# francescoalemanno/KissABC.jl

Hardware: AMD Instinct MI355X
Metric: walker proposal+cost evals/sec at N=65536 walkers, D=8 (higher is better)
Workload: dtype f64

## Files before the change

### include/kabc.h

```cpp
#ifndef KABC_H
#define KABC_H

#ifndef __HIPCC_RTC__
#include <stddef.h>
#include <stdint.h>
#else
#include "kabc_rtc_types.h"
#endif

#ifdef __cplusplus
extern "C" {
#endif

#define KABC_VERSION 321
#define KABC_MAX_DIM 16
#define KABC_MAX_DIM_DYN 256

typedef enum kabc_status {
    KABC_OK = 0,
    KABC_ERR_INVALID_ARG = 1,
    KABC_ERR_RETRY_EXHAUSTED = 2,
    KABC_ERR_INVALID_STATE = 3,
    KABC_ERR_DEVICE = 4,
    KABC_ERR_UNSUPPORTED = 5,
// ... 101 lines not shown

typedef struct kabc_reject_result {
    double* theta;
    double* cost;
    double* logprior;
    int64_t* index;
    int64_t capacity;
    int64_t n_out;
    int64_t draws;
    int64_t accepted_seen;
    double eps;
    int32_t exhausted;
    int32_t course;
    int64_t launches;
    double kernel_ms;
} kabc_reject_result_t;

void kabc_reject_default_opts(kabc_reject_opts_t* opts);
kabc_status_t kabc_abc_reject(kabc_ctx_t* ctx, const kabc_prior_t* prior, int32_t D, const kabc_cost_t* cost,
                              const kabc_reject_opts_t* opts, kabc_reject_result_t* result);

kabc_status_t kabc_abc_reject_batch(kabc_ctx_t* ctx, const kabc_prior_t* prior, int32_t D,
                                    const kabc_cost_t* costs, int64_t nruns, const uint64_t* seeds,
                                    const double* eps, const kabc_reject_opts_t* opts,
                                    kabc_reject_result_t* results, kabc_status_t* status);
void kabc_reject_batch_stats(int64_t out[4]);

kabc_status_t kabc_math_probe(kabc_ctx_t* ctx, int32_t fn, int64_t n, const double* x,
                              double* out);

kabc_status_t kabc_ais_wide_deal(const int32_t* simd, int32_t waves, int32_t chunk, int32_t nc,
                                 uint32_t* masks);
void kabc_ais_wide_shipped(int32_t geom[3]);

enum {
    KABC_PREBUILT_AIS_HALF = 1,
    KABC_PREBUILT_AIS_WIDE = 2,
    KABC_PREBUILT_AIS_SMALL = 3,
    KABC_PREBUILT_SMC_PHASES = 4,
    KABC_PREBUILT_SMC_LOOP = 5,
    KABC_PREBUILT_SMC_SMALL = 6,
    KABC_PREBUILT_ABCDE_GEN = 7,
    KABC_PREBUILT_ABCDE_SMALL = 8,
    KABC_PREBUILT_PF_PHASES = 9,
    KABC_PREBUILT_PF_SMALL = 10,
    KABC_PREBUILT_PF_BATCH = 11
};
int32_t kabc_prebuilt_has(int32_t family, int32_t cost_id, int32_t D, int32_t variant);
void kabc_ctx_last_kernel(kabc_ctx_t* ctx, int32_t info[6]);

kabc_status_t kabc_poison_probe(kabc_ctx_t* ctx, int64_t n, uint8_t* fresh, uint8_t* pooled,
                                uint8_t* recycled, int32_t info[2]);

kabc_status_t kabc_register_cost_plugin(const char* path, int32_t* out_cost_id);
kabc_status_t kabc_compile_cost_plugin(const char* src, const int32_t* dims, int32_t ndims,
                                       int32_t posterior_mask, int32_t* out_cost_id);
kabc_status_t kabc_plugin_precompile(int32_t cost_id, int32_t family, int32_t D, int32_t variant);

kabc_status_t kabc_compile_prior_plugin(const char* src, int32_t discrete, int32_t* out_kind);

kabc_status_t kabc_compile_mvprior_plugin(const char* src, int32_t* out_kind);

#define KABC_FAMILY_AIS 1
#define KABC_FAMILY_SMC 2
#define KABC_FAMILY_ABCDE 4
#define KABC_FAMILY_PFILTER 8
// ... 322 lines not shown
```

### kissabc.jl_amd/_cdefs.py

```python
import ctypes as C

KABC_MAX_DIM = 16
KABC_MAX_DIM_DYN = 256
KABC_VERSION = 321
KABC_COMM_ID_BYTES = 128
KABC_MAX_EXCHANGE_CHUNKS = 16
KABC_COMM_MAX_WORLD = 16
COMM_RCCL, COMM_P2P = 1, 2

KABC_OK, KABC_ERR_INVALID_ARG, KABC_ERR_RETRY_EXHAUSTED, KABC_ERR_INVALID_STATE, \
    KABC_ERR_DEVICE, KABC_ERR_UNSUPPORTED, KABC_ERR_NAN_COST, KABC_ERR_CANCELLED = range(8)

PRIOR_UNIFORM, PRIOR_NORMAL, PRIOR_TRUNCNORMAL, PRIOR_BETA, PRIOR_DISCRETE_UNIFORM, \
    PRIOR_NEGBINOMIAL, PRIOR_EXPONENTIAL, PRIOR_GAMMA, PRIOR_LOGNORMAL = range(1, 10)
PRIOR_USER_INIT = 10
PRIOR_MVNORMAL = 11
PRIOR_USER = 100
FAMILY_AIS, FAMILY_SMC, FAMILY_ABCDE, FAMILY_PFILTER, FAMILY_AIS_SMALL = 1, 2, 4, 8, 16

POSTERIOR_KERNELIZED, POSTERIOR_THRESHOLD, POSTERIOR_COMMON = 1, 2, 3
SUMMARY_AUTO, SUMMARY_FULL, SUMMARY_DIAG = 0, 1, 2
KABC_AUTOCORR_MAX_LAG = 256
KABC_HIST_MAX_BINS = 1024

# ... 97 lines not shown
                ("seed", C.c_uint64), ("first_row", C.c_int64)]


class RejectResult(C.Structure):
    _fields_ = [("theta", c_double_p), ("cost", c_double_p), ("logprior", c_double_p),
                ("index", C.POINTER(C.c_int64)), ("capacity", C.c_int64), ("n_out", C.c_int64),
                ("draws", C.c_int64), ("accepted_seen", C.c_int64), ("eps", C.c_double),
                ("exhausted", C.c_int32), ("course", C.c_int32), ("launches", C.c_int64),
                ("kernel_ms", C.c_double)]


ABI_REJECT_OPTS, ABI_REJECT_RESULT = 32, 33

VP = C.c_void_p
PROTOTYPES = {
    "kabc_version": (C.c_int32, []),
    "kabc_abi_sizeof": (C.c_int32, [C.c_int32]),
    "kabc_abi_offsetof": (C.c_int32, [C.c_int32, C.c_int32]),
    "kabc_mvnormal_register": (C.c_int, [c_double_p, c_double_p, C.c_int32, C.POINTER(C.c_int32)]),
    "kabc_last_error": (C.c_char_p, []),
    "kabc_device_count": (C.c_int32, []),
    "kabc_ctx_create": (C.c_int, [C.c_int32, VP, C.POINTER(VP)]),
    "kabc_ctx_destroy": (C.c_int, [VP]),
    "kabc_ctx_synchronize": (C.c_int, [VP]),
    "kabc_ctx_cancel": (C.c_int, [VP]),
    "kabc_ctx_clear_cancel": (C.c_int, [VP]),
    "kabc_ctx_cancel_on_sigint": (C.c_int, [VP, C.c_int32]),
    "kabc_math_probe": (C.c_int, [VP, C.c_int32, C.c_int64, c_double_p, c_double_p]),
    "kabc_poison_probe": (C.c_int, [VP, C.c_int64, C.POINTER(C.c_uint8), C.POINTER(C.c_uint8),
                                    C.POINTER(C.c_uint8), C.POINTER(C.c_int32)]),
    "kabc_ais_wide_deal": (C.c_int, [C.POINTER(C.c_int32), C.c_int32, C.c_int32, C.c_int32,
                                     C.POINTER(C.c_uint32)]),
    "kabc_ais_wide_shipped": (None, [C.POINTER(C.c_int32)]),
    "kabc_prebuilt_has": (C.c_int32, [C.c_int32, C.c_int32, C.c_int32, C.c_int32]),
    "kabc_ctx_last_kernel": (None, [VP, C.POINTER(C.c_int32)]),
    "kabc_host_alloc": (C.c_int, [C.c_size_t, C.POINTER(VP)]),
    "kabc_host_free": (C.c_int, [VP]),
    "kabc_factored_logpdf": (C.c_int, [VP, C.POINTER(Prior), C.c_int32, C.c_int64, c_double_p,
                                       c_double_p]),
    "kabc_factored_push_p": (C.c_int, [VP, C.POINTER(Prior), C.c_int32, C.c_int64, c_double_p,
                                       c_double_p]),
    "kabc_factored_rand": (C.c_int, [VP, C.POINTER(Prior), C.c_int32, C.c_uint64, C.c_uint32,
                                     C.c_int64, C.c_int64, C.c_uint64, c_double_p]),
    "kabc_cost_eval": (C.c_int, [VP, C.POINTER(Cost), C.c_int32, C.c_int64, c_double_p, C.c_int32,
                                 C.c_uint64, C.c_int64, c_double_p]),
    "kabc_prior_predictive": (C.c_int, [VP, C.POINTER(Prior), C.c_int32, C.POINTER(Cost), C.c_int64,
                                        C.c_int32, C.c_uint64, C.c_int64, c_double_p, c_double_p,
                                        c_double_p]),
    "kabc_eval_stats": (None, [c_double_p]),
    "kabc_reject_default_opts": (None, [C.POINTER(RejectOpts)]),
    "kabc_abc_reject": (C.c_int, [VP, C.POINTER(Prior), C.c_int32, C.POINTER(Cost), C.POINTER(RejectOpts),
                                  C.POINTER(RejectResult)]),
    "kabc_abc_reject_batch": (C.c_int, [VP, C.POINTER(Prior), C.c_int32, C.POINTER(Cost), C.c_int64,
                                        C.POINTER(C.c_uint64), c_double_p, C.POINTER(RejectOpts),
                                        C.POINTER(RejectResult), C.POINTER(C.c_int)]),
    "kabc_reject_batch_stats": (None, [C.POINTER(C.c_int64)]),
    "kabc_register_cost_plugin": (C.c_int, [C.c_char_p, C.POINTER(C.c_int32)]),
    "kabc_plugin_precompile": (C.c_int, [C.c_int32, C.c_int32, C.c_int32, C.c_int32]),
    "kabc_compile_cost_plugin": (C.c_int, [C.c_char_p, C.POINTER(C.c_int32), C.c_int32, C.c_int32,
                                         C.POINTER(C.c_int32)]),
    "kabc_compile_prior_plugin": (C.c_int, [C.c_char_p, C.c_int32, C.POINTER(C.c_int32)]),
    "kabc_compile_mvprior_plugin": (C.c_int, [C.c_char_p, C.POINTER(C.c_int32)]),
    "kabc_compile_model": (C.c_int, [C.POINTER(Model), C.c_int32, C.POINTER(C.c_int32)]),
    "kabc_model_release": (C.c_int, [C.c_int32]),
    "kabc_prefetch_model": (C.c_int, [C.POINTER(Model), C.c_int32]),
    "kabc_spec_counters": (C.c_int, [C.POINTER(C.c_uint64)]),
# ... 123 lines not shown
```

### kissabc.jl_amd/csrc/ais_kernels.hpp

```cpp
#pragma once

#include "kabc_device.hpp"
#ifndef __HIPCC_RTC__
#include "launcher.hpp"
#endif

namespace kabc {

struct AisArgs {
    double* x_act;
    const double* x_comp;
    double* lp;
    double* ll;
    double* trace;
    int32_t* dbg;
    DevCounters* counters;
    unsigned long long* slots;
    const double* cost_params;
    const double* cost_data;
    int64_t cost_ndata;
    int64_t row_first;
    int64_t rows_owned;
    int64_t n_comp;
    uint64_t seed;
    uint64_t t0;
    uint32_t id_base;
    int32_t nt;
    int32_t posterior;
    double eps;
    double reps;
    double box_lp;
    int32_t ablate;
    const PriorDev* prior;
    const uint64_t* seeds;
    int64_t stride_act, stride_comp, stride_own, stride_trace;
    const double* aux;
    int64_t stride_aux;
    int32_t dbg_nt, dbg_s0;
    int64_t params_stride, data_stride;
};

constexpr int ais_pre_blocks(int cost, int D) {
    const int n = cost >= KABC_COST_USER ? 0 : cost_pre_blocks(cost, D);
    return n <= 8 ? n : 0;
}

constexpr int kLateFrom = 10;
constexpr int kCounterSlots = 1024;

struct InitArgs {
    double* x_act;
    double* lp;
    double* ll;
    DevCounters* counters;
    const double* cost_params;
    const double* cost_data;
    int64_t cost_ndata;
    int64_t row_first;
    int64_t rows_owned;
    uint64_t seed;
    uint32_t id_base;
    int32_t posterior;
    int32_t cost_id;
    double eps;
    unsigned long long retry_budget;
// ... 79 lines not shown
#undef KABC_DEAL_UNROLL

template <int D>
struct RecGeom {
    static constexpr int NB = (D + 2) / 2;
    static constexpr int NZ = (D + 2 > 4) ? (D + 2) : 4;
};

template <int Q>
struct SubStepIx {
    static constexpr int value = Q;
};

template <int D, int CH>
struct RecBuf {
    uint32_t mva[CH][kBatch];
    uint32_t bb[CH][kBatch];
    uint32_t cc[CH][kBatch];
    double logu[CH][kBatch];
    double zs[CH][RecGeom<D>::NZ][kBatch];
};
template <int D>
using ChunkRec = RecBuf<D, kChunk>;

enum { kPriorBox = 0, kPriorSimple = 1, kPriorGeneral = 2, kPriorNormal = 3 };
constexpr int kPriorClasses = 4;
constexpr int kNbTabsGeneral = kNbLg1Block;

struct BoxPrior {
    const double* lo;
    const double* hi;
    uint32_t dmask;
    double lp;
};

#define KABC_BOXP(k) \
    "v_cmpx_ge_f64_e32 vcc, %[y" #k "], %[l" #k "]\n\tv_cmpx_le_f64_e32 vcc, %[y" #k "], %[h" #k "]\n\t"
#define KABC_BOXO(k) [y##k] "v"(y[k]), [l##k] "v"(lo[k]), [h##k] "v"(hi[k])
#if __has_builtin(__builtin_amdgcn_inverse_ballot_w64)
#define KABC_BOX_ASM(BODY, ...)                                                                   \
    unsigned long long saved, inside;                                                             \
    asm volatile("s_mov_b64 %[sv], exec\n\t" BODY "s_mov_b64 %[in], exec\n\ts_mov_b64 exec, %[sv]" \
                 : [in] "=&s"(inside), [sv] "=&s"(saved)                                          \
                 : __VA_ARGS__                                                                    \
                 : "vcc");                                                                        \
    return __builtin_amdgcn_inverse_ballot_w64(inside);
#else
#define KABC_BOX_ASM(BODY, ...)                                                                   \
    unsigned flag = 0;                                                                            \
    unsigned long long saved;                                                                     \
    asm volatile("s_mov_b64 %[sv], exec\n\t" BODY "v_mov_b32 %[fl], 1\n\ts_mov_b64 exec, %[sv]"  \
                 : [fl] "+v"(flag), [sv] "=&s"(saved)                                             \
                 : __VA_ARGS__                                                                    \
                 : "vcc");                                                                        \
    return flag != 0u;
#endif
template <int D>
__device__ __forceinline__ bool box_contains(const double* y, const double* lo, const double* hi);
template <>
__device__ __forceinline__ bool box_contains<2>(const double* y, const double* lo, const double* hi) {
    KABC_BOX_ASM(KABC_BOXP(0) KABC_BOXP(1), KABC_BOXO(0), KABC_BOXO(1))
}
template <>
__device__ __forceinline__ bool box_contains<3>(const double* y, const double* lo, const double* hi) {
    KABC_BOX_ASM(KABC_BOXP(0) KABC_BOXP(1) KABC_BOXP(2), KABC_BOXO(0), KABC_BOXO(1), KABC_BOXO(2))
}
template <>
__device__ __forceinline__ bool box_contains<4>(const double* y, const double* lo, const double* hi) {
    KABC_BOX_ASM(KABC_BOXP(0) KABC_BOXP(1) KABC_BOXP(2) KABC_BOXP(3), KABC_BOXO(0), KABC_BOXO(1), KABC_BOXO(2),
                 KABC_BOXO(3))
}
template <>
__device__ __forceinline__ bool box_contains<5>(const double* y, const double* lo, const double* hi) {
    KABC_BOX_ASM(KABC_BOXP(0) KABC_BOXP(1) KABC_BOXP(2) KABC_BOXP(3) KABC_BOXP(4), KABC_BOXO(0), KABC_BOXO(1),
                 KABC_BOXO(2), KABC_BOXO(3), KABC_BOXO(4))
}
template <>
__device__ __forceinline__ bool box_contains<6>(const double* y, const double* lo, const double* hi) {
    KABC_BOX_ASM(KABC_BOXP(0) KABC_BOXP(1) KABC_BOXP(2) KABC_BOXP(3) KABC_BOXP(4) KABC_BOXP(5), KABC_BOXO(0),
                 KABC_BOXO(1), KABC_BOXO(2), KABC_BOXO(3), KABC_BOXO(4), KABC_BOXO(5))
}
template <>
__device__ __forceinline__ bool box_contains<7>(const double* y, const double* lo, const double* hi) {
    KABC_BOX_ASM(KABC_BOXP(0) KABC_BOXP(1) KABC_BOXP(2) KABC_BOXP(3) KABC_BOXP(4) KABC_BOXP(5) KABC_BOXP(6),
                 KABC_BOXO(0), KABC_BOXO(1), KABC_BOXO(2), KABC_BOXO(3), KABC_BOXO(4), KABC_BOXO(5), KABC_BOXO(6))
}
template <>
__device__ __forceinline__ bool box_contains<8>(const double* y, const double* lo, const double* hi) {
    KABC_BOX_ASM(KABC_BOXP(0) KABC_BOXP(1) KABC_BOXP(2) KABC_BOXP(3) KABC_BOXP(4) KABC_BOXP(5) KABC_BOXP(6)
                     KABC_BOXP(7),
                 KABC_BOXO(0), KABC_BOXO(1), KABC_BOXO(2), KABC_BOXO(3), KABC_BOXO(4), KABC_BOXO(5), KABC_BOXO(6),
                 KABC_BOXO(7))
}
#undef KABC_BOX_ASM
#undef KABC_BOXO
#undef KABC_BOXP

template <int D, int COST, int PC>
__device__ __forceinline__ void loglike(const PriorDev* __restrict__ P, const BoxPrior& B,
                                        const GaussBoxPrior& GB,
                                        int posterior, double eps, double reps, const double* y,
                                        const double* cost_params, const double* cost_data,
                                        int64_t ndata, kabc_cost_rng_t* rng, double& lp,
                                        double& ll, bool& ev, const double* logtab = kabc_log_tab,
                                        const double* nbtab = nullptr) {
    double yp[D];
    constexpr bool kCheap = COST == KABC_COST_GAUSS_DIST || COST == KABC_COST_ROSENBROCK ||
                            COST == KABC_COST_DIRAC_SQ || COST == KABC_COST_ABS_DIFF ||
                            COST == KABC_COST_NORM_SHELL;
    if (posterior == KABC_POSTERIOR_COMMON) {
        lp = 0.0;
        ev = true;
        ll = eval_cost<COST, D>(y, cost_params, cost_data, ndata, rng);
        return;
    }
    if constexpr (PC == kPriorBox) {
        double lo[D], hi[D];
#pragma unroll
        for (int k = 0; k < D; ++k) {
            lo[k] = B.lo[k];
            hi[k] = B.hi[k];
        }
        bool in = true;
        if (__builtin_amdgcn_readfirstlane((int)B.dmask) == 0) {
            if constexpr (D >= 2 && D <= 8) in = box_contains<D>(y, lo, hi);
            else {
#pragma unroll
                for (int k = 0; k < D; ++k) in = in && (y[k] >= lo[k]) && (y[k] <= hi[k]);
            }
            if constexpr (kCheap) {
                lp = B.lp;
                ev = in;
                const double c = eval_cost<COST, D>(y, cost_params, cost_data, ndata, rng);
                if (posterior == KABC_POSTERIOR_KERNELIZED) {
                    const double q = kabc_div_rc(c, eps, reps);
                    ll = -0.5 * (q * q);
                } else {
                    ll = c;
                }
                return;
            }
#pragma unroll
            for (int k = 0; k < D; ++k) yp[k] = y[k];
        } else {
#pragma unroll
            for (int k = 0; k < D; ++k) {
                const double v = ((B.dmask >> k) & 1u) ? kabc_rint(y[k]) : y[k];
                yp[k] = v;
                in = in && (v >= lo[k]) && (v <= hi[k]);
            }
            if constexpr (kCheap) {
                lp = B.lp;
                ev = in;
                const double c = eval_cost<COST, D>(yp, cost_params, cost_data, ndata, rng);
                if (posterior == KABC_POSTERIOR_KERNELIZED) {
                    const double q = kabc_div_rc(c, eps, reps);
                    ll = -0.5 * (q * q);
                } else {
                    ll = c;
                }
                return;
            }
        }
        lp = in ? B.lp : -KABC_INF;
    } else if constexpr (PC == kPriorSimple || PC == kPriorNormal) {
        bool in;
        double sum;
        if constexpr (PC == kPriorNormal) sum = gaussbox_logpdf_push<D, true, false>(GB, y, yp, in);
        else if (__builtin_amdgcn_readfirstlane((int)GB.dmask) == 0) sum = gaussbox_logpdf_push<D, false, false>(GB, y, yp, in);
        else sum = gaussbox_logpdf_push<D, false, true>(GB, y, yp, in);
        lp = in ? sum : -KABC_INF;
    } else {
#ifdef KABC_MODEL_SPEC
        if constexpr (D == kabc_mspec::D) lp = model_logpdf_push<D, kNbTabsGeneral>(y, yp, logtab, nbtab);
        else
#endif
        lp = factored_logpdf_push<D, false>(P, y, yp, logtab, nbtab);
    }
    ev = kabc_isfinite(lp);
    if (posterior == KABC_POSTERIOR_KERNELIZED) {
        if constexpr (kCheap) {
            const double c = eval_cost<COST, D>(yp, cost_params, cost_data, ndata, rng);
            const double q = kabc_div_rc(c, eps, reps);
            ll = ev ? -0.5 * (q * q) : lp;
        } else {
            ll = lp;
            if (ev) {
                const double c = eval_cost<COST, D>(yp, cost_params, cost_data, ndata, rng);
                const double q = kabc_div_rc(c, eps, reps);
                ll = -0.5 * (q * q);
            }
        }
    } else {
        if constexpr (kCheap) {
            const double c = eval_cost<COST, D>(yp, cost_params, cost_data, ndata, rng);
            ll = ev ? c : -lp;
        } else {
            ll = -lp;
            if (ev) ll = eval_cost<COST, D>(yp, cost_params, cost_data, ndata, rng);
        }
    }
}

#ifdef KABC_PROBES
#define KABL A.ablate
#else
#define KABL 0
#endif
struct NoMid {
    __device__ __forceinline__ void operator()() const {}
};
template <int D, class Mid = NoMid, bool WALK = true, class Rec = ChunkRec<D>, class Args = AisArgs>
// ... 187 lines not shown
    const int nchunks = (A.nt + CH - 1) / CH;
    const bool consumer = G::kWide ? wave < NBAT : wave == 0;
    const bool tprobe = (KABL & 128) && A.dbg;
    unsigned long long t_begin = 0, t_bar = 0;
    if (tprobe) t_begin = __builtin_amdgcn_s_memtime();
#define KABC_TIMED_BARRIER()                                              \
    do {                                                                  \
        if (tprobe) {                                                     \
            const unsigned long long tb_ = __builtin_amdgcn_s_memtime(); \
            __syncthreads();                                              \
            t_bar += __builtin_amdgcn_s_memtime() - tb_;                  \
        } else {                                                          \
            __syncthreads();                                              \
        }                                                                 \
    } while (0)

    auto comp_row = [&](uint32_t idx) -> const double* {
        return reinterpret_cast<const double*>(reinterpret_cast<const char*>(A.x_comp) +
                                               (size_t)(idx * (uint32_t)(D * sizeof(double))));
    };
    const bool active = consumer && (lane < n_active);
    const int64_t r = r0 + lane;
    const int64_t row = A.row_first + r;
    double x[D];
    double lp = 0.0, ll = 0.0;
    unsigned int n_eval = 0, n_acc = 0;
    int err = 0;
    if (active) {
        load_row<D>(A.x_act + row * D, x);
        lp = A.lp[r];
        ll = A.ll[r];
        if (!ld_valid(PK, lp, ll)) err = 2;
    }

    static_assert(KABC_MATH_TAB_WORDS == 2 * kAisBlock && (G::kBlock == kAisBlock || G::kBlock >= 2 * kAisBlock),
                  "two table words per thread, or one for each of the first 512");
    const bool tab_thread = G::kBlock <= KABC_MATH_TAB_WORDS || threadIdx.x < (unsigned)KABC_MATH_TAB_WORDS;
    const double tab0 = tab_thread ? kabc_log_tab[threadIdx.x] : 0.0;
    [[maybe_unused]] double tab1 = 0.0;
    if constexpr (G::kBlock == kAisBlock) tab1 = kabc_log_tab[threadIdx.x + kAisBlock];
    if (threadIdx.x < D * (int)(sizeof(PriorDev) / 8))
        reinterpret_cast<double*>(sprior)[threadIdx.x] =
            reinterpret_cast<const double*>(A.prior)[threadIdx.x];
    if (threadIdx.x < D) {
        sbox_lo[threadIdx.x] = A.prior[threadIdx.x].p[0];
        sbox_hi[threadIdx.x] = A.prior[threadIdx.x].p[1];
    }
    uint32_t dmask = 0, gmask = 0;
    for (int k = 0; k < D; ++k) {
        dmask |= (A.prior[k].discrete ? 1u : 0u) << k;
        gmask |= (gaussbox_is_gauss(A.prior[k].kind) ? 1u : 0u) << k;
    }
    if constexpr (kGaussBox) {
        if (threadIdx.x < D) gaussbox_stage(sgb[threadIdx.x], A.prior[threadIdx.x]);
    }
    const GaussBoxPrior gbox = {sgb, gmask, dmask};
    constexpr bool kBoxRegs = (PC == kPriorBox) && D <= 8;
    double blo[kBoxRegs ? D : 1], bhi[kBoxRegs ? D : 1];
    const BoxPrior box = {kBoxRegs ? blo : sbox_lo, kBoxRegs ? bhi : sbox_hi, dmask, A.box_lp};

    [[maybe_unused]] kabc_u128_t pro01[2] = {};
    if constexpr (!G::kWide) {
        if (wave > 0 && wave - 1 < A.nt && lane < n_active) {
            const uint32_t w = w_base + (uint32_t)lane;
            const uint64_t t = A.t0 + (uint64_t)(wave - 1);
            pro01[0] = kabc_stream_block(A.seed, w, t, 0u, KABC_DOM_AIS_MOVE);
            pro01[1] = kabc_stream_block(A.seed, w, t, 1u, KABC_DOM_AIS_MOVE);
        }
    }
    if (tab_thread) slogtab[threadIdx.x] = tab0;
    if constexpr (G::kBlock == kAisBlock) slogtab[threadIdx.x + kAisBlock] = tab1;
    if constexpr (G::kWide) {
        uint32_t hw;
        asm volatile("s_getreg_b32 %0, hwreg(HW_REG_HW_ID)" : "=s"(hw));
        if (lane == 0) ssimd[wave] = (hw >> 4) & 3u;
    }
#ifdef KABC_MODEL_SPEC
    [[maybe_unused]] const bool nb_on = kNbTabs > 0;
#else
    [[maybe_unused]] const bool nb_on = kNbTabs > 0 && A.nt >= 8;
#endif
    if constexpr (kNbTabs > 0) {
        static_assert(kNbEntries == kAisBlock, "one table entry per thread (of the first 256)");
        const bool nb_thread = !G::kWide || threadIdx.x < (unsigned)kNbEntries;
        int slot = 0;
        bool has_nb = false;
        for (int k = 0; k < D; ++k) {
            if (A.prior[k].kind == KABC_PRIOR_NEGBINOMIAL) {
                has_nb = true;
                if (nb_on && slot < kNbTabs) {
                    if (nb_thread)
                        snb[slot * kNbEntries + threadIdx.x] =
// ... 151 lines not shown
                            const double W = xa[k] * Z;
                            y[k] = pa[k] + W;
                        }
                    }
                    if (move == 2u) {
                        const double gamma = zs[0];
#pragma unroll
                        for (int k = 0; k < D; ++k) {
                            const double Wk = (pa[k] - pb[k]) * gamma;
                            const double sk = kabc_fabs(pa[k] - pb[k]) + kabc_fabs(x[k] - pb[k]) +
                                              kabc_fabs(xa[k]);
                            const double Tk = kabc_div_rc(gamma * sk, 300.0, 1.0 / 300.0) * zs[1 + k];
                            y[k] = x[k] + Wk + Tk;
                        }
                    }
                    __builtin_amdgcn_sched_barrier(0);
                    if constexpr (kLate) {
                        load_row<D>(comp_row(mvan & 0x3fffffffu), na);
                        load_row<D>(comp_row(bn), nb);
                    }
                    kabc_cost_rng_t rng = {A.seed, t, w_base + (uint32_t)lane, KABC_DOM_AIS_COST, 0u,
                                           0u, nullptr, slogtab};
                    if constexpr (kAuxW > 0) {
                        rng.aux = &saux[(KABL & 2) ? 0 : (c & 1)][bmine][si][0][lane];
                        rng.aux_stride = kBatch;
                    }
                    if constexpr (kPre > 0) {
                        rng.pre = &spre[(KABL & 2) ? 0 : (c & 1)][bmine][si][0][lane];
                        rng.pre_n = (uint32_t)kPre;
                        rng.pre_stride = (uint32_t)kBatch;
                    }
                    double nlp, nll;
                    bool ev;
                    loglike<D, COST, PC>(sprior, box, gbox, PK, A.eps, A.reps, y, cparams,
                                         A.cost_data, A.cost_ndata, &rng, nlp, nll, ev, slogtab,
                                         kNbTabs > 0 ? snb : nullptr);
                    __builtin_amdgcn_sched_barrier(0);
                    n_eval += ev ? 1u : 0u;
                    const bool valid = ev && ld_valid(PK, nlp, nll);
                    const double e = -logu;
                    bool acc;
                    if (PK == KABC_POSTERIOR_KERNELIZED) {
                        const double lW = corr + (nlp + nll) - (lp + ll);
                        acc = valid && (-e <= lW);
                    } else if (PK == KABC_POSTERIOR_COMMON) {
                        const double lW = corr + nll - ll;
                        acc = valid && (-e <= lW);
                    } else {
                        const double lW = corr + nlp - lp;
                        const double mx = (A.eps > ll) ? A.eps : ll;
                        const double lW2 = mx - nll;
                        acc = valid && (-e <= lW) && (lW2 >= 0.0);
                    }
                    if (acc) {
#pragma unroll
                        for (int k = 0; k < D; ++k) x[k] = y[k];
                        lp = nlp;
                        ll = nll;
                        n_acc += 1u;
                    }
#pragma unroll
                    for (int k = 0; k < D; ++k) asm volatile("" : "+v"(x[k]));
                    if (dbg_on) {
                        int32_t* d = A.dbg + (r * A.dbg_nt + (A.dbg_s0 + s0 + si)) * 6;
                        d[0] = (int32_t)move;
                        d[1] = acc ? 1 : 0;
                        d[2] = (int32_t)(mva & 0x3fffffffu);
                        d[3] = move >= 2u ? (int32_t)R.bb[si][lane] : -1;
                        d[4] = move == 3u ? (int32_t)R.cc[si][lane] : -1;
                        d[5] = ev ? 1 : 0;
                    }
                };
                static_assert(CH >= 1 && CH <= 8, "the consumer spells out up to 8 sub-steps");
                auto sub_even = [&](auto SI) __attribute__((always_inline)) {
                    if constexpr (decltype(SI)::value < CH) {
                        if constexpr (kLate) substep(SI, r0a, r0b, r0a, r0b);
                        else substep(SI, r0a, r0b, r1a, r1b);
                    }
                };
                auto sub_odd = [&](auto SI) __attribute__((always_inline)) {
                    if constexpr (decltype(SI)::value < CH) {
                        if constexpr (kLate) substep(SI, r0a, r0b, r0a, r0b);
                        else substep(SI, r1a, r1b, r0a, r0b);
                    }
                };
                sub_even(SubStepIx<0>{});
                if (ns > 1) sub_odd(SubStepIx<1>{});
                if (ns > 2) sub_even(SubStepIx<2>{});
                if constexpr (CH > 3) {
                    if (ns > 3) sub_odd(SubStepIx<3>{});
                    if (ns > 4) sub_even(SubStepIx<4>{});
                    if (ns > 5) sub_odd(SubStepIx<5>{});
                    if (ns > 6) sub_even(SubStepIx<6>{});
                    if (ns > 7) sub_odd(SubStepIx<7>{});
                }
            }
            KABC_TIMED_BARRIER();
        }
    }

    if (tprobe && lane == 0) {
        const unsigned long long t_end = __builtin_amdgcn_s_memtime();
        int32_t* d = A.dbg + (r0_wg * A.nt) * 6 + 2 * (NBAT + NPROD) + wave * 2;
        d[0] = (int32_t)(t_end - t_begin);
        d[1] = (int32_t)t_bar;
    }
    if ((KABL & 64) && A.dbg && lane == 0) {
        uint32_t hw;
        asm volatile("s_getreg_b32 %0, hwreg(HW_REG_HW_ID)" : "=s"(hw));
        A.dbg[(r0_wg * A.nt) * 6 + wave] = (int32_t)hw;
    }
    if (consumer) {
        if (active) {
            store_row<D>(A.x_act + row * D, x);
            A.lp[r] = lp;
            A.ll[r] = ll;
            if (A.trace) {
                double xp[D];
#pragma unroll
                for (int k = 0; k < D; ++k)
                    xp[k] = (sprior[k].discrete && PK != KABC_POSTERIOR_COMMON)
                                ? kabc_rint(x[k]) : x[k];
                store_row<D>(A.trace + r * D, xp);
            }
        }
        const unsigned long long se = wave_total_u32(n_eval);
        const unsigned long long sa = wave_total_u32(n_acc);
        if (lane == 0 && (!G::kWide || n_active > 0)) {
            unsigned long long* sl =
                A.slots + (size_t)((blockIdx.x * NBAT + bmine + blockIdx.y * gridDim.x * NBAT) & (kCounterSlots - 1)) * 8;
            atomicAdd(&sl[0], (unsigned long long)n_active * (unsigned long long)A.nt);
            atomicAdd(&sl[1], se);
            atomicAdd(&sl[2], sa);
        }
        if (err) atomicMax(&A.counters->error, err);
    }
#undef KABC_TIMED_BARRIER
}

template <int D, int COST, int PC, int PK>
__global__ void __launch_bounds__(kAisBlock) __attribute__((amdgpu_waves_per_eu(2, 2)))
ais_half_kernel(const AisArgs A0) {
    ais_half_body<D, COST, PC, PK, HalfGeom>(A0);
}

template <int D, int COST, int PC, int PK, int K, int NC, int W = 8, bool ONE = (W > 8)>
__global__ void __launch_bounds__(W * 64) __attribute__((amdgpu_waves_per_eu(W / 4, W / 4)))
// ... 109 lines not shown
```

### kissabc.jl_amd/csrc/capi_ais.hip

```cpp
#include <chrono>
#include <condition_variable>
#include <cstdio>
#include <cstdlib>
#include <mutex>
#include <thread>
#include <type_traits>
#include <vector>

#include "ais_aux_kernels.hpp"
#include "ais_dyn_kernels.hpp"
#include "ais_dyn_small_kernel.hpp"
#include "ais_small_kernel.hpp"
#include "ais_summary_host.hpp"
#include "host_common.hpp"
#include "plugin_registry.hpp"

namespace kabc {

#define KABC_DECL_COST(id)                                                \
    AisLaunchFn find_ais_kernel_cost_##id(int D, int pc);                 \
    AisLaunchFn find_ais_kernel_cost_##id##_nrm(int D, int pc);           \
    AisLaunchFn find_ais_kernel_cost_##id##_hi(int D, int pc);            \
    AisLaunchFn find_ais_wide_kernel_cost_##id(int D, int pc);            \
    AisLaunchFn find_ais_wide_kernel_cost_##id##_nrm(int D, int pc);      \
// ... 158 lines not shown
    kabc_prior_t* d_raw = nullptr;
    double* d_scratch = nullptr;
    int32_t nchains = 1;
    uint64_t* d_seeds = nullptr;
    unsigned long long* d_chain_retries = nullptr;
    uint32_t id_base[2] = {};
    double* d_half[2] = {};
    bool own_halves = false;
    double* d_lp[2] = {};
    double* d_ll[2] = {};
    DevCounters* d_counters = nullptr;
    unsigned long long* d_slots = nullptr;
    PriorDev* d_prior = nullptr;
    uint64_t seed = 0, t = 0;
    int32_t rank = 0, world = 1;
    AisLaunch launch;
    AisLaunch launch_wide;
    int32_t pc = 0;
    int32_t half_pcx = -1;
    bool small_ok = false;
    AisSmallLaunch small;
    int32_t small_pcx = 0;
    AisDynSmallLaunchFn dsmall = nullptr;
    AisDynSmallPlan dplan;
    double* d_strace = nullptr;
    size_t strace_cap = 0;
    ModelUnit* unit = nullptr;
    int32_t spec_state = KABC_SPEC_NONE;
    int32_t spec_variant = 0;
    int64_t launches = 0;
    int64_t spec_switch_at = -1;
    std::chrono::steady_clock::time_point spec_next_poll;
    double box_lp = 0.0;
    bool initialised = false;
    double* d_trace[kTraceBufs] = {};
    size_t trace_cap[kTraceBufs] = {};
    hipStream_t copy_stream = nullptr;
    hipEvent_t ev_filled[kTraceBufs] = {};
    double* d_aux = nullptr;
    size_t aux_cap = 0;
    hipEvent_t ev_blk[2] = {};
    AisSummary sum;
    int32_t* d_dbg = nullptr;
    int64_t dbg_cap = 0;
    bool timing = false;
    int32_t timing_stride = 1;
    int32_t open_count = 0;
    std::vector<hipEvent_t> ev;
    std::vector<int32_t> ev_n;
    size_t ev_used = 0;
    kabc_stats_t last = {};
    struct XT {
        hipEvent_t e0, e1, e2;
        hipEvent_t x0[KABC_MAX_EXCHANGE_CHUNKS], x1[KABC_MAX_EXCHANGE_CHUNKS];
        bool closed;
    };
    std::vector<XT> xt;
    size_t xt_used = 0;
    int xt_open = -1;
};

static constexpr size_t kXtHalves = 128;

static kabc_status_t check_handle(const kabc_ais_t* h) {
    if (!h) {
        set_error("AIS handle is NULL");
// ... 139 lines not shown
    }
    if (m->posterior != KABC_POSTERIOR_KERNELIZED && m->posterior != KABC_POSTERIOR_THRESHOLD &&
        m->posterior != KABC_POSTERIOR_COMMON) {
        set_error("unknown posterior kind %d", m->posterior);
        return KABC_ERR_INVALID_ARG;
    }
    if (world < 1 || rank < 0 || rank >= world ||
        (!comm && world > 1 && n_total % (2 * world) != 0)) {
        set_error("sharded AIS needs nparticles divisible by 2*world (got %lld, world %d)",
                  (long long)n_total, world);
        return KABC_ERR_INVALID_ARG;
    }
    if (!cost_dim_ok_rt(m->cost.id, m->D)) {
        set_error("DeviceCost id %d does not accept D = %d", m->cost.id, m->D);
        return KABC_ERR_UNSUPPORTED;
    }
    {
        int n_user = 0;
        for (int k = 0; k < m->D; ++k) n_user += m->prior[k].kind == KABC_PRIOR_USER_INIT;
        if (n_user) {
            const CostPlugin* pl = find_plugin(m->cost.id);
            if (n_user != m->D || m->posterior != KABC_POSTERIOR_COMMON || dyn || !pl || !pl->has_sample_init) {
                set_error("KABC_PRIOR_USER_INIT: every component must carry it, the model must be a "
                          "CommonLogDensity of at most %d parameters, and its log-density a user cost "
                          "whose snippet defines KABC_USER_SAMPLE_INIT + kabc_user_sample_init",
                          KABC_MAX_DIM);
                return KABC_ERR_INVALID_ARG;
            }
        }
    }
    return KABC_OK;
}

static kabc_status_t ais_prepare_prior(kabc_ais_t* h, const kabc_model_t* m) {
    const bool dyn = h->D > KABC_MAX_DIM;
    bool prior_ok = true;
    if (dyn) {
        h->raw_dyn.assign(m->prior, m->prior + m->D);
        h->prior_dyn.resize((size_t)m->D);
        for (int k = 0; k < m->D && prior_ok; ++k)
            prior_ok = prepare_prior(h->raw_dyn[k], h->prior_dyn[k]);
    } else {
        std::memcpy(h->raw, m->prior, sizeof(kabc_prior_t) * m->D);
        prior_ok = prepare_priors(h->raw, h->D, h->prior);
    }
    if (!prior_ok) {
        set_error("invalid prior parameters");
        return KABC_ERR_INVALID_ARG;
    }
    bool isbox = true, gaussbox = true, allnormal = true;
    for (int k = 0; k < m->D; ++k) {
        const int kd = m->prior[k].kind;
        const bool box = kd == KABC_PRIOR_UNIFORM || kd == KABC_PRIOR_DISCRETE_UNIFORM;
        const bool gauss = kd == KABC_PRIOR_NORMAL || kd == KABC_PRIOR_TRUNCNORMAL;
        isbox = isbox && box;
        gaussbox = gaussbox && (box || gauss);
        allnormal = allnormal && kd == KABC_PRIOR_NORMAL;
    }
    h->pc = isbox ? kPriorBox : allnormal ? kPriorNormal : gaussbox ? kPriorSimple : kPriorGeneral;
    static_assert(kPriorClasses == 4, "capi_plugin.hip decodes pcx with 4 prior classes");
    h->box_lp = h->prior.c[0].c0;
    for (int k = 1; k < h->D && !dyn; ++k) h->box_lp += h->prior.c[k].c0;
    return KABC_OK;
}

static kabc_status_t ais_resolve_kernels(kabc_ais_t* h, const kabc_model_t* m) {
    const bool dyn = h->D > KABC_MAX_DIM;
    KABC_HIP_CHECK(hipSetDevice(h->ctx->device));
    if (kabc_status_t st = model_unit_for(m->prior, m->D, m->cost.id, &h->unit)) return st;
    ModelUnit* unit = h->unit;
    if (dyn) {
        if (unit) {
            const PluginKernel kh = unit_kernel(unit, kPfAisDyn, m->D, 0), ki = unit_kernel(unit, kPfAisDyn, m->D, 1);
            h->dyn = AisDynLaunch(kh.mod, unit_kernel(unit, kPfAisDyn, m->D, 2).mod, unit_kernel(unit, kPfAisDyn, m->D, 3).mod, ki.mod);
            if (!h->dyn) return KABC_ERR_DEVICE;
        } else if (m->cost.id >= KABC_COST_USER) {
            const CostPlugin* pl = find_plugin(m->cost.id);
            if (pl && pl->rtc) {
                const PluginKernel kh = plugin_kernel(pl, kPfAisDyn, m->D, 0), ki = plugin_kernel(pl, kPfAisDyn, m->D, 1);
                h->dyn = AisDynLaunch(kh.mod, plugin_kernel(pl, kPfAisDyn, m->D, 2).mod, plugin_kernel(pl, kPfAisDyn, m->D, 3).mod, ki.mod);
            } else if (pl && pl->ais_dyn) {
                h->dyn = AisDynLaunch((AisDynLaunchFn)pl->ais_dyn());
            }
        } else {
            h->dyn = AisDynLaunch(find_ais_dyn_kernel(m->cost.id));
        }
        if (!h->dyn) {
            if (!get_error()[0])
                set_error("length(prior) = %d > %d: no run-time-dimension kernels for cost id %d (a plugin .so "
                          "built from older headers?)", m->D, KABC_MAX_DIM, m->cost.id);
            return KABC_ERR_UNSUPPORTED;
        }
    }
    const char* e = std::getenv("KABC_AIS_SMALL");
    const bool off = e && e[0] == '0', asked = e && e[0] == '1';
// ... 140 lines not shown
    if (c.error == 1) {
        set_error("ld_correction is invalid");
        return KABC_ERR_INVALID_STATE;
    }
    if (c.error == 2) {
        set_error("starting sample invalid.");
        return KABC_ERR_INVALID_STATE;
    }
    return KABC_OK;
}

template <class A>
static void fill_args(A& a, const kabc_ais_t* h) {
    constexpr bool aux = std::is_same_v<A, AuxArgs>, init = std::is_same_v<A, InitArgs>;
    constexpr bool dyn = std::is_same_v<A, AisDynArgs>, small = std::is_same_v<A, AisSmallArgs>;
    constexpr bool dsm = std::is_same_v<A, AisDynSmallArgs>;
    std::memset(&a, 0, sizeof a);
    a.cost_params = h->d_cost_params;
    a.cost_data = h->d_cost_data;
    a.cost_ndata = h->cost_ndata;
    a.seed = h->seed;
    a.seeds = h->d_seeds;
    if constexpr (!aux) {
        a.counters = h->d_counters;
        a.eps = h->eps;
    }
    if constexpr (init) a.prior = h->prior;
    if constexpr (!aux && !init) {
        a.slots = h->d_slots;
        a.reps = (h->posterior == KABC_POSTERIOR_COMMON) ? 1.0 : 1.0 / h->eps;
        a.prior = h->d_prior;
    }
    if constexpr (!aux && !dyn && !dsm && !init) a.box_lp = h->box_lp;
    if constexpr (!aux && !small) a.posterior = h->posterior;
    if constexpr (dyn || dsm || init) a.cost_id = h->cost_id;
    if constexpr (dyn || dsm) a.D = h->D;
    a.params_stride = h->params_stride;
    if constexpr (!aux) a.data_stride = h->data_stride;
}

template <class T>
static kabc_status_t grow(kabc_ais_t* h, T** p, size_t* cap, size_t bytes) {
    if (bytes <= *cap) return KABC_OK;
    if (*p) {
        KABC_HIP_CHECK(hipStreamSynchronize(h->ctx->stream));
        KABC_HIP_CHECK(hipFree(*p));
        *p = nullptr;
        *cap = 0;
    }
    KABC_HIP_CHECK(dev_malloc(p, bytes));
    *cap = bytes;
    return KABC_OK;
}

static int64_t enqueue_aux(kabc_ais_t* h, int half, int64_t row_first, int64_t rows, uint64_t t0, int32_t nt,
                           double* base) {
    AuxArgs x;
    fill_args(x, h);
    x.aux = base;
    x.row_first = row_first;
    x.rows = rows;
    x.t0 = t0;
    x.id_base = h->id_base[half];
    x.nt = nt;
    x.stride_aux = (int64_t)nt * aux_prepass_words(h->cost_id) * rows;
    launch_aux_prepass(h->cost_id, x, h->ctx->stream, (unsigned)h->nchains);
// ... 464 lines not shown
                a.aux = h->d_aux;
                a.stride_aux = enqueue_aux(h, half, sg.first, sg.count, a.t0, nb, h->d_aux);
            }
            const bool wide = ais_use_wide(h, sg.count, nb);
            (wide ? h->launch_wide : h->launch)(a, s, (unsigned)h->nchains);
            const int pcl = h->half_pcx % kPriorClasses;
            note_kernel(h->ctx, h->half_pcx >= 0, wide ? KABC_PREBUILT_AIS_WIDE : KABC_PREBUILT_AIS_HALF, h->cost_id,
                        h->D, pcl, h->posterior, wide ? ais_wide_waves_c(h->D, pcl) : kAisBlock / kWave);
        }
    }
    if (t_on && ++h->open_count >= h->timing_stride)
        if (kabc_status_t st = timing_close_pair(h)) return st;
    KABC_HIP_CHECK(hipGetLastError());
    return KABC_OK;
}

kabc_status_t kabc_ais_wide_deal(const int32_t* simd, int32_t waves, int32_t chunk, int32_t nc,
                                 uint32_t* masks) {
    if (!simd || !masks || (waves != 8 && waves != 12) || chunk < 1 || chunk > 8 || nc > chunk) {
        set_error("kabc_ais_wide_deal: bad argument (waves 8 or 12, chunk 1..8, nc <= chunk)");
        return KABC_ERR_INVALID_ARG;
    }
    uint64_t sd = 0;
    for (int w = 0; w < waves; ++w) {
        if (simd[w] < 0 || simd[w] > 15) {
            set_error("kabc_ais_wide_deal: SIMD id %d of wave %d is not in 0..15", (int)simd[w], w);
            return KABC_ERR_INVALID_ARG;
        }
        sd |= (uint64_t)simd[w] << (4 * w);
    }
    for (int p = 0; p < waves - kWideBatches; ++p) masks[p] = wide_deal_mask(sd, waves, chunk, nc, p);
    return KABC_OK;
}
void kabc_ais_wide_shipped(int32_t geom[3]) {
    geom[0] = kWideW;
    geom[1] = kWideK;
    geom[2] = kWideNC;
}

kabc_status_t kabc_ais_half_generation(kabc_ais_t* h, int32_t half, int32_t ntransitions,
                                       void* dev_trace_rows) {
    if (check_handle(h)) return KABC_ERR_INVALID_ARG;
    if (!h->initialised) {
        set_error("kabc_ais_init / kabc_ais_set_state has not been called");
        return KABC_ERR_INVALID_STATE;
    }
    if ((half != 0 && half != 1) || ntransitions < 1) {
        set_error("half must be 0/1 and ntransitions >= 1");
        return KABC_ERR_INVALID_ARG;
    }
    if (kabc_status_t st = counter_room(h, 1, ntransitions, "kabc_ais_half_generation")) return st;
    for (const kabc_ais::Seg& sg : h->seg[half])
        if (kabc_status_t st = launch_half_seg(h, half, sg, ntransitions, (double*)dev_trace_rows))
            return st;
    return KABC_OK;
}

kabc_status_t kabc_ais_end_generation(kabc_ais_t* h, int32_t ntransitions) {
    if (check_handle(h)) return KABC_ERR_INVALID_ARG;
    if (kabc_status_t st = counter_room(h, 1, ntransitions, "kabc_ais_end_generation")) return st;
    h->t += (uint64_t)ntransitions;
    return KABC_OK;
}

}

// ... 856 lines not shown
```

Before: 32.90 billion.

## Trim AIS box-prior inner loop with symmetric-box abs test and scalar eval counting

```diff
diff --git a/include/kabc.h b/include/kabc.h
--- a/include/kabc.h
+++ b/include/kabc.h
@@ -157,6 +157,8 @@
 kabc_status_t kabc_ais_wide_deal(const int32_t* simd, int32_t waves, int32_t chunk, int32_t nc,
                                  uint32_t* masks);
 void kabc_ais_wide_shipped(int32_t geom[3]);
+
+kabc_status_t kabc_ais_box_sym(const kabc_prior_t* prior, int32_t D, int32_t* sym);
 
 enum {
     KABC_PREBUILT_AIS_HALF = 1,
diff --git a/kissabc.jl_amd/_cdefs.py b/kissabc.jl_amd/_cdefs.py
--- a/kissabc.jl_amd/_cdefs.py
+++ b/kissabc.jl_amd/_cdefs.py
@@ -153,6 +153,7 @@
     "kabc_ais_wide_deal": (C.c_int, [C.POINTER(C.c_int32), C.c_int32, C.c_int32, C.c_int32,
                                      C.POINTER(C.c_uint32)]),
     "kabc_ais_wide_shipped": (None, [C.POINTER(C.c_int32)]),
+    "kabc_ais_box_sym": (C.c_int, [C.POINTER(Prior), C.c_int32, C.POINTER(C.c_int32)]),
     "kabc_prebuilt_has": (C.c_int32, [C.c_int32, C.c_int32, C.c_int32, C.c_int32]),
     "kabc_ctx_last_kernel": (None, [VP, C.POINTER(C.c_int32)]),
     "kabc_host_alloc": (C.c_int, [C.c_size_t, C.POINTER(VP)]),
diff --git a/kissabc.jl_amd/csrc/ais_kernels.hpp b/kissabc.jl_amd/csrc/ais_kernels.hpp
--- a/kissabc.jl_amd/csrc/ais_kernels.hpp
+++ b/kissabc.jl_amd/csrc/ais_kernels.hpp
@@ -31,6 +31,7 @@
     double reps;
     double box_lp;
     int32_t ablate;
+    int32_t box_sym;
     const PriorDev* prior;
     const uint64_t* seeds;
     int64_t stride_act, stride_comp, stride_own, stride_trace;
@@ -176,11 +177,21 @@
     const double* hi;
     uint32_t dmask;
     double lp;
+    uint32_t sym;
 };
+
+inline bool box_is_symmetric(const double* lo, const double* hi, uint32_t dmask, int D) {
+    if (dmask != 0u || D < 2 || D > 8) return false;
+    for (int k = 0; k < D; ++k)
+        if (!(lo[k] == -hi[k])) return false;
+    return true;
+}
 
 #define KABC_BOXP(k) \
     "v_cmpx_ge_f64_e32 vcc, %[y" #k "], %[l" #k "]\n\tv_cmpx_le_f64_e32 vcc, %[y" #k "], %[h" #k "]\n\t"
 #define KABC_BOXO(k) [y##k] "v"(y[k]), [l##k] "v"(lo[k]), [h##k] "v"(hi[k])
+#define KABC_BOXS(k) "v_cmpx_le_f64_e64 vcc, |%[y" #k "]|, %[h" #k "]\n\t"
+#define KABC_BOXSO(k) [y##k] "v"(y[k]), [h##k] "v"(hi[k])
 #if __has_builtin(__builtin_amdgcn_inverse_ballot_w64)
 #define KABC_BOX_ASM(BODY, ...)                                                                   \
     unsigned long long saved, inside;                                                             \
@@ -188,7 +199,8 @@
                  : [in] "=&s"(inside), [sv] "=&s"(saved)                                          \
                  : __VA_ARGS__                                                                    \
                  : "vcc");                                                                        \
-    return __builtin_amdgcn_inverse_ballot_w64(inside);
+    return inside;
+#define KABC_BOX_LANE(m) __builtin_amdgcn_inverse_ballot_w64(m)
 #else
 #define KABC_BOX_ASM(BODY, ...)                                                                   \
     unsigned flag = 0;                                                                            \
@@ -197,57 +209,102 @@
                  : [fl] "+v"(flag), [sv] "=&s"(saved)                                             \
                  : __VA_ARGS__                                                                    \
                  : "vcc");                                                                        \
-    return flag != 0u;
+    return __builtin_amdgcn_ballot_w64(flag != 0u);
+#define KABC_BOX_LANE(m) \
+    ((((m) >> __builtin_amdgcn_mbcnt_hi(~0u, __builtin_amdgcn_mbcnt_lo(~0u, 0u))) & 1ull) != 0ull)
 #endif
 template <int D>
-__device__ __forceinline__ bool box_contains(const double* y, const double* lo, const double* hi);
-template <>
-__device__ __forceinline__ bool box_contains<2>(const double* y, const double* lo, const double* hi) {
+__device__ __forceinline__ unsigned long long box_contains(const double* y, const double* lo, const double* hi);
+template <>
+__device__ __forceinline__ unsigned long long box_contains<2>(const double* y, const double* lo, const double* hi) {
     KABC_BOX_ASM(KABC_BOXP(0) KABC_BOXP(1), KABC_BOXO(0), KABC_BOXO(1))
 }
 template <>
-__device__ __forceinline__ bool box_contains<3>(const double* y, const double* lo, const double* hi) {
+__device__ __forceinline__ unsigned long long box_contains<3>(const double* y, const double* lo, const double* hi) {
     KABC_BOX_ASM(KABC_BOXP(0) KABC_BOXP(1) KABC_BOXP(2), KABC_BOXO(0), KABC_BOXO(1), KABC_BOXO(2))
 }
 template <>
-__device__ __forceinline__ bool box_contains<4>(const double* y, const double* lo, const double* hi) {
+__device__ __forceinline__ unsigned long long box_contains<4>(const double* y, const double* lo, const double* hi) {
     KABC_BOX_ASM(KABC_BOXP(0) KABC_BOXP(1) KABC_BOXP(2) KABC_BOXP(3), KABC_BOXO(0), KABC_BOXO(1), KABC_BOXO(2),
                  KABC_BOXO(3))
 }
 template <>
-__device__ __forceinline__ bool box_contains<5>(const double* y, const double* lo, const double* hi) {
+__device__ __forceinline__ unsigned long long box_contains<5>(const double* y, const double* lo, const double* hi) {
     KABC_BOX_ASM(KABC_BOXP(0) KABC_BOXP(1) KABC_BOXP(2) KABC_BOXP(3) KABC_BOXP(4), KABC_BOXO(0), KABC_BOXO(1),
                  KABC_BOXO(2), KABC_BOXO(3), KABC_BOXO(4))
 }
 template <>
-__device__ __forceinline__ bool box_contains<6>(const double* y, const double* lo, const double* hi) {
+__device__ __forceinline__ unsigned long long box_contains<6>(const double* y, const double* lo, const double* hi) {
     KABC_BOX_ASM(KABC_BOXP(0) KABC_BOXP(1) KABC_BOXP(2) KABC_BOXP(3) KABC_BOXP(4) KABC_BOXP(5), KABC_BOXO(0),
                  KABC_BOXO(1), KABC_BOXO(2), KABC_BOXO(3), KABC_BOXO(4), KABC_BOXO(5))
 }
 template <>
-__device__ __forceinline__ bool box_contains<7>(const double* y, const double* lo, const double* hi) {
+__device__ __forceinline__ unsigned long long box_contains<7>(const double* y, const double* lo, const double* hi) {
     KABC_BOX_ASM(KABC_BOXP(0) KABC_BOXP(1) KABC_BOXP(2) KABC_BOXP(3) KABC_BOXP(4) KABC_BOXP(5) KABC_BOXP(6),
                  KABC_BOXO(0), KABC_BOXO(1), KABC_BOXO(2), KABC_BOXO(3), KABC_BOXO(4), KABC_BOXO(5), KABC_BOXO(6))
 }
 template <>
-__device__ __forceinline__ bool box_contains<8>(const double* y, const double* lo, const double* hi) {
+__device__ __forceinline__ unsigned long long box_contains<8>(const double* y, const double* lo, const double* hi) {
     KABC_BOX_ASM(KABC_BOXP(0) KABC_BOXP(1) KABC_BOXP(2) KABC_BOXP(3) KABC_BOXP(4) KABC_BOXP(5) KABC_BOXP(6)
                      KABC_BOXP(7),
                  KABC_BOXO(0), KABC_BOXO(1), KABC_BOXO(2), KABC_BOXO(3), KABC_BOXO(4), KABC_BOXO(5), KABC_BOXO(6),
                  KABC_BOXO(7))
 }
+template <int D>
+__device__ __forceinline__ unsigned long long box_contains_sym(const double* y, const double* hi);
+template <>
+__device__ __forceinline__ unsigned long long box_contains_sym<2>(const double* y, const double* hi) {
+    KABC_BOX_ASM(KABC_BOXS(0) KABC_BOXS(1), KABC_BOXSO(0), KABC_BOXSO(1))
+}
+template <>
+__device__ __forceinline__ unsigned long long box_contains_sym<3>(const double* y, const double* hi) {
+    KABC_BOX_ASM(KABC_BOXS(0) KABC_BOXS(1) KABC_BOXS(2), KABC_BOXSO(0), KABC_BOXSO(1), KABC_BOXSO(2))
+}
+template <>
+__device__ __forceinline__ unsigned long long box_contains_sym<4>(const double* y, const double* hi) {
+    KABC_BOX_ASM(KABC_BOXS(0) KABC_BOXS(1) KABC_BOXS(2) KABC_BOXS(3), KABC_BOXSO(0), KABC_BOXSO(1), KABC_BOXSO(2),
+                 KABC_BOXSO(3))
+}
+template <>
+__device__ __forceinline__ unsigned long long box_contains_sym<5>(const double* y, const double* hi) {
+    KABC_BOX_ASM(KABC_BOXS(0) KABC_BOXS(1) KABC_BOXS(2) KABC_BOXS(3) KABC_BOXS(4), KABC_BOXSO(0), KABC_BOXSO(1),
+                 KABC_BOXSO(2), KABC_BOXSO(3), KABC_BOXSO(4))
+}
+template <>
+__device__ __forceinline__ unsigned long long box_contains_sym<6>(const double* y, const double* hi) {
+    KABC_BOX_ASM(KABC_BOXS(0) KABC_BOXS(1) KABC_BOXS(2) KABC_BOXS(3) KABC_BOXS(4) KABC_BOXS(5), KABC_BOXSO(0),
+                 KABC_BOXSO(1), KABC_BOXSO(2), KABC_BOXSO(3), KABC_BOXSO(4), KABC_BOXSO(5))
+}
+template <>
+__device__ __forceinline__ unsigned long long box_contains_sym<7>(const double* y, const double* hi) {
+    KABC_BOX_ASM(KABC_BOXS(0) KABC_BOXS(1) KABC_BOXS(2) KABC_BOXS(3) KABC_BOXS(4) KABC_BOXS(5) KABC_BOXS(6),
+                 KABC_BOXSO(0), KABC_BOXSO(1), KABC_BOXSO(2), KABC_BOXSO(3), KABC_BOXSO(4), KABC_BOXSO(5), KABC_BOXSO(6))
+}
+template <>
+__device__ __forceinline__ unsigned long long box_contains_sym<8>(const double* y, const double* hi) {
+    KABC_BOX_ASM(KABC_BOXS(0) KABC_BOXS(1) KABC_BOXS(2) KABC_BOXS(3) KABC_BOXS(4) KABC_BOXS(5) KABC_BOXS(6)
+                     KABC_BOXS(7),
+                 KABC_BOXSO(0), KABC_BOXSO(1), KABC_BOXSO(2), KABC_BOXSO(3), KABC_BOXSO(4), KABC_BOXSO(5), KABC_BOXSO(6),
+                 KABC_BOXSO(7))
+}
 #undef KABC_BOX_ASM
+#undef KABC_BOXSO
+#undef KABC_BOXS
 #undef KABC_BOXO
 #undef KABC_BOXP
 
-template <int D, int COST, int PC>
+constexpr bool ais_trim_c(int cost, int D, int pc, bool regs168) {
+    return pc == kPriorBox && D >= 2 && D <= 8 && !(regs168 && D == 8 && cost == KABC_COST_GAUSS_DIST);
+}
+
+template <int D, int COST, int PC, bool TRIM = false>
 __device__ __forceinline__ void loglike(const PriorDev* __restrict__ P, const BoxPrior& B,
                                         const GaussBoxPrior& GB,
                                         int posterior, double eps, double reps, const double* y,
                                         const double* cost_params, const double* cost_data,
                                         int64_t ndata, kabc_cost_rng_t* rng, double& lp,
                                         double& ll, bool& ev, const double* logtab = kabc_log_tab,
-                                        const double* nbtab = nullptr) {
+                                        const double* nbtab = nullptr, unsigned long long* evm = nullptr) {
     double yp[D];
     constexpr bool kCheap = COST == KABC_COST_GAUSS_DIST || COST == KABC_COST_ROSENBROCK ||
                             COST == KABC_COST_DIRAC_SQ || COST == KABC_COST_ABS_DIFF ||
@@ -266,15 +323,20 @@
             hi[k] = B.hi[k];
         }
         bool in = true;
+        [[maybe_unused]] unsigned long long inm = 0;
         if (__builtin_amdgcn_readfirstlane((int)B.dmask) == 0) {
-            if constexpr (D >= 2 && D <= 8) in = box_contains<D>(y, lo, hi);
-            else {
+            if constexpr (D >= 2 && D <= 8) {
+                if (TRIM && __builtin_amdgcn_readfirstlane((int)B.sym) != 0) inm = box_contains_sym<D>(y, hi);
+                else inm = box_contains<D>(y, lo, hi);
+                in = KABC_BOX_LANE(inm);
+            } else {
 #pragma unroll
                 for (int k = 0; k < D; ++k) in = in && (y[k] >= lo[k]) && (y[k] <= hi[k]);
             }
             if constexpr (kCheap) {
                 lp = B.lp;
                 ev = in;
+                if constexpr (TRIM) *evm = inm;
                 const double c = eval_cost<COST, D>(y, cost_params, cost_data, ndata, rng);
                 if (posterior == KABC_POSTERIOR_KERNELIZED) {
                     const double q = kabc_div_rc(c, eps, reps);
@@ -296,6 +358,7 @@
             if constexpr (kCheap) {
                 lp = B.lp;
                 ev = in;
+                if constexpr (TRIM) *evm = __builtin_amdgcn_ballot_w64(in);
                 const double c = eval_cost<COST, D>(yp, cost_params, cost_data, ndata, rng);
                 if (posterior == KABC_POSTERIOR_KERNELIZED) {
                     const double q = kabc_div_rc(c, eps, reps);
@@ -322,6 +385,7 @@
         lp = factored_logpdf_push<D, false>(P, y, yp, logtab, nbtab);
     }
     ev = kabc_isfinite(lp);
+    if constexpr (TRIM) *evm = __builtin_amdgcn_ballot_w64(ev);
     if (posterior == KABC_POSTERIOR_KERNELIZED) {
         if constexpr (kCheap) {
             const double c = eval_cost<COST, D>(yp, cost_params, cost_data, ndata, rng);
@@ -575,6 +639,10 @@
         ll = A.ll[r];
         if (!ld_valid(PK, lp, ll)) err = 2;
     }
+    constexpr bool kTrim = ais_trim_c(COST, D, PC, G::kWide && G::kOneRowSet) && PK != KABC_POSTERIOR_COMMON;
+    [[maybe_unused]] double lsum = lp + ll;
+    constexpr bool kLpOfBox = kTrim && PK == KABC_POSTERIOR_KERNELIZED;
+    constexpr bool kSumState = kTrim && PK == KABC_POSTERIOR_KERNELIZED;
 
     static_assert(KABC_MATH_TAB_WORDS == 2 * kAisBlock && (G::kBlock == kAisBlock || G::kBlock >= 2 * kAisBlock),
                   "two table words per thread, or one for each of the first 512");
@@ -600,7 +668,8 @@
     const GaussBoxPrior gbox = {sgb, gmask, dmask};
     constexpr bool kBoxRegs = (PC == kPriorBox) && D <= 8;
     double blo[kBoxRegs ? D : 1], bhi[kBoxRegs ? D : 1];
-    const BoxPrior box = {kBoxRegs ? blo : sbox_lo, kBoxRegs ? bhi : sbox_hi, dmask, A.box_lp};
+    const BoxPrior box = {kBoxRegs ? blo : sbox_lo, kBoxRegs ? bhi : sbox_hi, dmask, A.box_lp,
+                          (uint32_t)A.box_sym};
 
     [[maybe_unused]] kabc_u128_t pro01[2] = {};
     if constexpr (!G::kWide) {
@@ -818,16 +887,26 @@
                     }
                     double nlp, nll;
                     bool ev;
-                    loglike<D, COST, PC>(sprior, box, gbox, PK, A.eps, A.reps, y, cparams,
-                                         A.cost_data, A.cost_ndata, &rng, nlp, nll, ev, slogtab,
-                                         kNbTabs > 0 ? snb : nullptr);
+                    [[maybe_unused]] unsigned long long evm = 0;
+                    loglike<D, COST, PC, kTrim>(sprior, box, gbox, PK, A.eps, A.reps, y, cparams,
+                                                A.cost_data, A.cost_ndata, &rng, nlp, nll, ev, slogtab,
+                                                kNbTabs > 0 ? snb : nullptr, &evm);
                     __builtin_amdgcn_sched_barrier(0);
-                    n_eval += ev ? 1u : 0u;
+                    if constexpr (!kTrim) {
+                        n_eval += ev ? 1u : 0u;
+                    } else {
+                        unsigned long long cout;
+                        asm("v_addc_co_u32_e64 %[n], %[co], 0, %[n], %[m]"
+                            : [n] "+v"(n_eval), [co] "=&s"(cout)
+                            : [m] "s"(evm));
+                    }
                     const bool valid = ev && ld_valid(PK, nlp, nll);
                     const double e = -logu;
                     bool acc;
+                    [[maybe_unused]] double nsum = 0.0;
                     if (PK == KABC_POSTERIOR_KERNELIZED) {
-                        const double lW = corr + (nlp + nll) - (lp + ll);
+                        nsum = nlp + nll;
+                        const double lW = kSumState ? corr + nsum - lsum : corr + nsum - (lp + ll);
                         acc = valid && (-e <= lW);
                     } else if (PK == KABC_POSTERIOR_COMMON) {
                         const double lW = corr + nll - ll;
@@ -841,8 +920,9 @@
                     if (acc) {
 #pragma unroll
                         for (int k = 0; k < D; ++k) x[k] = y[k];
-                        lp = nlp;
+                        if constexpr (!kLpOfBox) lp = nlp;
                         ll = nll;
+                        if constexpr (kSumState) lsum = nsum;
                         n_acc += 1u;
                     }
 #pragma unroll
@@ -899,6 +979,9 @@
     if (consumer) {
         if (active) {
             store_row<D>(A.x_act + row * D, x);
+            if constexpr (kLpOfBox) {
+                if (n_acc != 0u) lp = A.box_lp;
+            }
             A.lp[r] = lp;
             A.ll[r] = ll;
             if (A.trace) {
diff --git a/kissabc.jl_amd/csrc/capi_ais.hip b/kissabc.jl_amd/csrc/capi_ais.hip
--- a/kissabc.jl_amd/csrc/capi_ais.hip
+++ b/kissabc.jl_amd/csrc/capi_ais.hip
@@ -214,6 +214,7 @@
     int64_t spec_switch_at = -1;
     std::chrono::steady_clock::time_point spec_next_poll;
     double box_lp = 0.0;
+    int32_t box_sym = 0;
     bool initialised = false;
     double* d_trace[kTraceBufs] = {};
     size_t trace_cap[kTraceBufs] = {};
@@ -419,6 +420,19 @@
     return KABC_OK;
 }
 
+static int32_t box_symmetric(const PriorDev* c, int D) {
+    if (D < 1 || D > KABC_MAX_DIM) return 0;
+    double lo[KABC_MAX_DIM], hi[KABC_MAX_DIM];
+    uint32_t dmask = 0;
+    for (int k = 0; k < D; ++k) {
+        if (c[k].kind != KABC_PRIOR_UNIFORM && c[k].kind != KABC_PRIOR_DISCRETE_UNIFORM) return 0;
+        lo[k] = c[k].p[0];
+        hi[k] = c[k].p[1];
+        dmask |= (c[k].discrete ? 1u : 0u) << k;
+    }
+    return box_is_symmetric(lo, hi, dmask, D) ? 1 : 0;
+}
+
 static kabc_status_t ais_prepare_prior(kabc_ais_t* h, const kabc_model_t* m) {
     const bool dyn = h->D > KABC_MAX_DIM;
     bool prior_ok = true;
@@ -448,6 +462,7 @@
     static_assert(kPriorClasses == 4, "capi_plugin.hip decodes pcx with 4 prior classes");
     h->box_lp = h->prior.c[0].c0;
     for (int k = 1; k < h->D && !dyn; ++k) h->box_lp += h->prior.c[k].c0;
+    h->box_sym = (!dyn && h->pc == kPriorBox) ? box_symmetric(h->prior.c, h->D) : 0;
     return KABC_OK;
 }
 
@@ -654,6 +669,7 @@
         a.prior = h->d_prior;
     }
     if constexpr (!aux && !dyn && !dsm && !init) a.box_lp = h->box_lp;
+    if constexpr (std::is_same_v<A, AisArgs>) a.box_sym = h->box_sym;
     if constexpr (!aux && !small) a.posterior = h->posterior;
     if constexpr (dyn || dsm || init) a.cost_id = h->cost_id;
     if constexpr (dyn || dsm) a.D = h->D;
@@ -1184,6 +1200,15 @@
     for (int p = 0; p < waves - kWideBatches; ++p) masks[p] = wide_deal_mask(sd, waves, chunk, nc, p);
     return KABC_OK;
 }
+kabc_status_t kabc_ais_box_sym(const kabc_prior_t* prior, int32_t D, int32_t* sym) {
+    PriorSet ps;
+    if (!sym || !prepare_priors(prior, D, ps)) {
+        set_error("kabc_ais_box_sym: bad argument (D 1..%d components with valid parameters)", KABC_MAX_DIM);
+        return KABC_ERR_INVALID_ARG;
+    }
+    *sym = box_symmetric(ps.c, D);
+    return KABC_OK;
+}
 void kabc_ais_wide_shipped(int32_t geom[3]) {
     geom[0] = kWideW;
     geom[1] = kWideK;
```

New measurement: 33.41 billion, median of 6. 1.02x the previous value.
